# samuel-vitorino/sopro

Measured on AMD Instinct MI355X. Metric: audio_seconds_per_second, higher is better.
Workload: dtype f32; 1 GPU; Sopro-135M synthesize, 32 utterances x 200 frames per GPU (BASELINE configs[1]), S=64 text tokens, 32 distinct 150-frame reference voice(s) per batch prepared outside the timed region, top_p=0.9 T=1.05 anti_loop (reference defaults), synthetic weights with EOS suppressed; batch_per_gpu=32, frames=200, voices_per_batch=32, parallelism=replicas x1 (utterance sharding, no collective), lanes_per_gpu=4

## Files before the change

include/sopro_hip.h:

```cpp
#ifndef SOPRO_HIP_H
#define SOPRO_HIP_H

#include <stdint.h>

#ifdef __cplusplus
extern "C" {
#endif

#define SOPRO_ABI_VERSION 42

const char* sopro_last_error(void);
int sopro_abi_version(void);
int sopro_build_flags(void);
int sopro_set_lds_floor(int bytes);
int sopro_set_host_wait(int blocking);
int sopro_device_info(int device, int* out4);

int sopro_capture_begin(void* stream);
int sopro_capture_end(void* stream, void** graph_exec_out);
int sopro_graph_launch(void* graph_exec, void* stream);
int sopro_graph_launch_n(void* graph_exec, void* stream, int32_t n);
int sopro_graph_destroy(void* graph_exec);
int sopro_stream_create_cu_range(int first_cu, int n_cus, void** stream_out);
int sopro_stream_create_cu_mask(const uint32_t* mask, int32_t words, void** stream_out);
// ... 70 lines not shown
  long long* dbg;
  float eps;
  int32_t B, N, K, epilogue;
  int32_t ring_len, ring_bcap, dil, ksize;
  int32_t np, ksplit, rms_norm;
  int32_t w_layout;
  const float* aux_W; const float* aux_bias; const float* aux_R; float* aux_Y;
  int64_t aux_ldy, aux_ldr, aux_y_part_stride;
  int32_t aux_tiles, aux_flags;
  int32_t ring_format;
  int32_t mt, nt;
} sopro_skinny_args;
int sopro_skinny_f32(const sopro_skinny_args* args, void* stream);
int sopro_pack_skinny_w(const float* W, int64_t ldw, int32_t N, int32_t K, int32_t glu, float* out, void* stream);
int64_t sopro_skinny_packed_floats(int32_t N, int32_t K, int32_t glu);
int sopro_pack_skinny_w_bf16(const float* W, int64_t ldw, int32_t N, int32_t K, int32_t glu, void* out, void* stream);

int sopro_fill2d_u32(void* p, int64_t pitch, int32_t rows, int32_t width, uint32_t value, void* stream);
int sopro_copy2d_u32(void* dst, int64_t dpitch, const void* src, int64_t spitch, int32_t rows, int32_t width, void* stream);
int sopro_nar_seed_i32(int32_t* tokens, int32_t Q, const int32_t* cb0, int64_t cb0_bstride, int32_t B, int32_t T, int32_t vmax, void* stream);
int sopro_cvt_f32_bf16(const float* src, void* dst, int64_t n, void* stream);
int sopro_cvt_bf16_f32(const void* src, float* dst, int64_t n, void* stream);
enum { SOPRO_NORM_RMS = 0, SOPRO_NORM_LN = 1 };
int sopro_norm_f32(const float* x, int64_t ldx, int64_t x_seg_stride , float* out, int64_t ldo, const float* w, const float* b,
                   const float* mul, const float* add, int32_t rows, int32_t rows_per_seg, int32_t C,
                   float eps, int32_t kind, void* stream);
int sopro_row_stats_f32(const float* x, int64_t ldx, int64_t x_seg_stride , int32_t rows, int32_t rows_per_seg, int32_t C,
                        float* stats, void* stream);
int sopro_rms_match_f32(const float* a, const float* x, float* out, int32_t rows, int32_t C, void* stream);
int sopro_tanh_affine_f32(const float* in, float* out, float c0, float c1, int64_t n, void* stream);
int sopro_add_pos_f32(const float* rowvec, const float* table, float* out, int32_t B, int32_t T, int32_t C,
                      int32_t pos0, void* stream);
int sopro_masked_mean_f32(const float* x, const int32_t* lens, float* out, int32_t B, int32_t T, int32_t C,
                          void* stream);

int sopro_stats_pool_f32(const float* h, const float* logit, const int32_t* lens, float* out, int32_t B, int32_t T,
                         int32_t C, void* stream);
int sopro_l2norm_f32(const float* x, float* out, int32_t rows, int32_t C, float eps, void* stream);

int sopro_dwconv_f32(const float* x, const float* w, const float* bias, const float* res, float* out,
                     const int32_t* lens, int32_t B, int32_t T, int32_t C, int32_t ksize, int32_t dil,
                     int32_t left, int32_t mode, void* stream);

int sopro_codebook_sum_f32(const int32_t* tok, int32_t ldt, const int32_t* col, const int32_t* off, const float* wq,
                           int32_t nq, const float* table, int64_t table_rows, const float* base, float alpha,
                           float beta, float* out, int64_t ldo, int64_t o_seg_stride, int32_t rows,
                           int32_t rows_per_seg, int32_t D, void* stream);
int sopro_text_embed_f32(const int32_t* ids, const int32_t* lens, const float* table, int64_t table_rows,
                         const float* pe, float* out, int32_t B, int32_t T, int32_t C, void* stream);
int sopro_argmax_rows_f32(const float* x, int64_t ldx, int32_t* out, int64_t ldo, int32_t inner, int32_t rows, int32_t N,
                          void* stream);
int sopro_argmax_partials_i32(const float* partials, int64_t ldp, int32_t* out, int64_t ldo, int32_t heads, int32_t per_head, int32_t V,
                              int32_t rows, void* stream);

int sopro_fir1_f32(const float* x, int64_t x_seg_stride, int32_t n_in, const float* w, const float* bias, float* out,
                   int64_t ldo, int64_t o_seg_stride, int32_t B, int32_t n_out, int32_t C, int32_t K, int32_t stride,
                   int32_t left, void* stream);
int sopro_rvq_assign_f32(const float* scores, int64_t lds, int32_t V, const float* table, float* res, int64_t ldr,
                         int32_t D, int32_t* codes, int64_t ldc, int32_t rows, void* stream);

typedef struct sopro_attn_args {
  const float* Q; int64_t ldq; int64_t q_bstride;
  const float* K; int64_t ldk; int64_t k_bstride;
  const float* V; int64_t ldv; int64_t v_bstride;
  float* O; int64_t ldo; int64_t o_bstride;
  const int32_t* klens;
  int32_t B, H, dh, Tq, Tk;
  int32_t causal, q_pos0, k_pos0, window;
  float scale;
  const int32_t* kv_index;
} sopro_attn_args;
int sopro_attention_f32(const sopro_attn_args* args, void* stream);
int sopro_attention_split_bf16(const sopro_attn_args* args, int32_t passes, void* stream);
int sopro_attn_decode_f32(const sopro_attn_args* args, void* stream);
typedef struct sopro_xattn_args {
  const float* X; int64_t ldx;
  const float* Xp; int64_t xp_stride;
  const float* norm_w;
  const float* Kp; const float* Vp;
  const int32_t* klens;
  float* Y; int64_t y_part_stride;
  float eps, gate, scale;
  int32_t np, B, H, D, S_cap;
  const float* Qp; int64_t qp_stride;
  int32_t nqp, k_unfolded;
  int32_t kv_format;
} sopro_xattn_args;
int sopro_xattn_step_f32(const sopro_xattn_args* args, void* stream);

int sopro_rope_f32(float* x, int64_t ldx, const float* cos_t, const float* sin_t, int32_t rows,
                   int32_t rows_per_seg, int32_t pos0, int32_t H, int32_t dh, void* stream);

int sopro_upsample2_f32(const float* x, const float* w, float* y, int64_t y_seg_stride, int32_t B, int32_t T,
                        int32_t C, void* stream);
int sopro_final_conv_f32(const float* h, int64_t h_seg_stride, const float* w, float bias, float* wav,
                         int64_t wav_seg_stride, int32_t B, int32_t T, void* stream);

int sopro_seanet_tail_f32(const float* h, int64_t h_seg_stride, const float* w1, const float* b1, const float* w2,
                          const float* b2, const float* wf, float bf, float* wav, int64_t wav_seg_stride, int32_t B,
                          int32_t T, void* stream);
int sopro_seanet_tail_p_f32(const float* h, int64_t h_seg_stride, const float* w1, const float* b1, const float* w2,
                            const float* b2, const float* wf, float bf, float* wav, int64_t wav_seg_stride, int32_t B,
                            int32_t T, int32_t passes, void* stream);
int sopro_seanet_res128_f32(const float* h, int64_t h_seg_stride, const float* w1, const float* b1, const float* w2, const float* b2,
                            float* out, int64_t out_seg_stride, int32_t B, int32_t T, void* stream);
int sopro_seanet_res128_p_f32(const float* h, int64_t h_seg_stride, const float* w1, const float* b1, const float* w2, const float* b2,
// ... 214 lines not shown
```

sopro_amd/csrc/stages.hip:

```cpp
#include <stdlib.h>

#include <algorithm>
#include <map>
#include <string>
#include <vector>

#include "common.h"

int sopro_stream_batch_append(float* cur, float* other, const float* qkv, int32_t hs, int32_t rows, int64_t bstride, int32_t n, int32_t kv_len,
                              int32_t nkeep, hipStream_t s);
int sopro_stream_batch_gather(float* kv, const int32_t* keep, int32_t n_keep, int32_t layers, int32_t rows_cap, int64_t bstride, int32_t hs, int32_t half,
                              int32_t kv_len, hipStream_t s);

namespace {

struct Ten {
  const void* p = nullptr;
  int64_t shape[4] = {0, 0, 0, 0};
  int ndim = 0;
  const float* f() const { return reinterpret_cast<const float*>(p); }
};

struct Wt {
  const float* f32 = nullptr;
// ... 886 lines not shown
  for (int i = 0; i < c.n_layers_ar; ++i) {
    const int64_t n = (int64_t)((c.ar_kernel - 1) * c.ar_dilations[i] + 1) * B * D;
    STG(sopro_fill2d_u32(p.rings[i], n, 1, (int32_t)n, 0u, s));
  }
  STG(sopro_fill2d_u32(p.hist, (int64_t)B * Tar, 1, B * Tar, 0u, s));
  for (int k = 0; k < 8; ++k) {
    uint32_t u;
    memcpy(&u, &params[k], 4);
    STG(sopro_fill2d_u32(p.params + k, 1, 1, 1, u, s));
  }
  STG(sopro_fill2d_u32(p.nonce, B, 1, B, nonce, s));
  STG(sopro_fill2d_u32(p.key, 1, 1, 1, (uint32_t)seed, s));
  STG(sopro_fill2d_u32(p.key + 1, 1, 1, 1, (uint32_t)(seed >> 32), s));
  sopro_ar_state& st = p.st;
  memset(&st, 0, sizeof(st));
  st.x_cur = p.x[0]; st.cond = p.cond; st.emb = F(e, "cb_embed"); st.hist = p.hist;
  st.step = p.ctr; st.row_step = p.row_step; st.n_stopped = p.ctr + 2;
  st.first_eos = p.first_eos; st.stop_t = p.stop_t; st.recent = p.recent; st.params = p.params; st.nonce = p.nonce;
  st.key = p.key; st.seed = 0; st.B = B; st.D = D; st.Tar = Tar; st.max_steps = Tar; st.V = c.codebook_size; st.bos_row = c.bos_row;
  STG(sopro_ar_init(&st, s));
  if (p.graph && (p.graph_B != B || p.graph_S_cap != p.S_cap || p.graph_Tar != Tar || p.graph_ws != workspace)) {
    STG(sopro_graph_destroy(p.graph));
    p.graph = nullptr;
  }
  return 0;
}

int sopro_ar_run_graph(sopro_engine* e, int32_t n_steps, void* stream) {
  SOPRO_CHECK_ARG(e && e->ar.ws && n_steps >= 0 && stream, "sopro_ar_begin first; a non-default stream is needed for graph capture");
  ArPlan& p = e->ar;
  if (!p.graph) {
    STG(sopro_capture_begin(stream));
    const int rc = ar_issue_step(e, (hipStream_t)stream);
    void* g = nullptr;
    const int rc2 = sopro_capture_end(stream, &g);
    if (rc != 0) return rc;
    if (rc2 != 0) return rc2;
    p.graph = g; p.graph_B = p.B; p.graph_S_cap = p.S_cap; p.graph_Tar = p.Tar; p.graph_ws = p.ws;
  }
  for (int i = 0; i < n_steps; ++i) STG(sopro_graph_launch(p.graph, stream));
  return 0;
}

int sopro_ar_tokens(sopro_engine* e, int32_t* hist, int32_t* first_eos, int32_t* n_stopped, void* stream) {
  SOPRO_CHECK_ARG(e && e->ar.ws, "sopro_ar_begin first");
  hipStream_t s = (hipStream_t)stream;
  const ArPlan& p = e->ar;
  if (hist) STG(sopro_copy2d_u32(hist, (int64_t)p.B * p.Tar, p.hist, (int64_t)p.B * p.Tar, 1, p.B * p.Tar, s));
  if (first_eos) STG(sopro_copy2d_u32(first_eos, p.B, p.first_eos, p.B, 1, p.B, s));
  if (n_stopped) STG(sopro_copy2d_u32(n_stopped, 1, p.ctr + 2, 1, 1, 1, s));
  return 0;
}

struct NarWs { float *xa, *xb, *h, *x1, *u, *z, *part, *cond; int32_t *lens, *range; SplitK sk; };
static size_t nar_carve(const sopro_engine* e, NarWs& w, void* ws, int B, int T) {
  const sopro_engine_cfg& c = e->c;
  const size_t M = (size_t)B * T, D = c.d_model;
  int nh_max = 0;
  for (int i = 0; i < c.n_stages; ++i) nh_max = c.stage_n_cb[i] > nh_max ? c.stage_n_cb[i] : nh_max;
  Carver cv(ws);
  w.xa = cv.take<float>(M * D); w.xb = cv.take<float>(M * D); w.h = cv.take<float>(M * D); w.x1 = cv.take<float>(M * D);
  w.u = cv.take<float>(M * 4 * D); w.z = cv.take<float>(M * c.nar_head_dim);
  w.part = cv.take<float>(M * nh_max * (c.codebook_size / 64) * 2);
  w.cond = cv.take<float>(M * D);
  w.lens = cv.take<int32_t>(B);
  w.range = cv.take<int32_t>(4);
  w.sk.tickets = cv.take<int32_t>(SPLITK_TICKETS);
  w.sk.ws = M <= 1024 ? cv.take<float>(SPLITK_WS_BYTES / 4) : nullptr;
  return cv.off;
}

int64_t sopro_nar_workspace_bytes(const sopro_engine* e, int32_t B, int32_t T) {
  if (!e || B <= 0 || T <= 0) return 0;
  NarWs w;
  return (int64_t)nar_carve(e, w, nullptr, B, T);
}

static int ssm_block_bufs(sopro_engine* e, hipStream_t s, float* h, float* x1, float* u, const SplitK* sk, const float* x, float* out,
                          const std::string& p, int B, int T, int ksize, int dil, const int32_t* lens, const char* sfx, int32_t* range) {
  const int D = e->c.d_model, M = B * T;
  const int total = (ksize - 1) * dil, left = total / 2;
  G g; g.M = M; g.N = 2 * D; g.K = D; g.bias = F(e, p + ".glu.b"); g.epi = SOPRO_EPI_GLU; g.rms_eps = RMS_EPS; g.range_events = range;
  STG(gemm(s, x, WT(e, p + ".glu.wn" + sfx), nullptr, h, g));
  STG(sopro_dwconv_f32(h, F(e, p + ".dw.w"), F(e, p + ".dw.b"), x, x1, lens, B, T, D, ksize, dil, left, 1, s));
  G f1; f1.M = M; f1.N = 4 * D; f1.K = D; f1.bias = F(e, p + ".ff1.b"); f1.epi = SOPRO_EPI_GELU; f1.rms_eps = RMS_EPS; f1.range_events = range;
  STG(gemm(s, x1, WT(e, p + ".ff1.wn" + sfx), nullptr, u, f1));
  G f2; f2.M = M; f2.N = D; f2.K = 4 * D; f2.bias = F(e, p + ".ff2.b"); f2.epi = SOPRO_EPI_RES; f2.R = x1; f2.sk = sk; f2.range_events = range;
  return gemm(s, u, WT(e, p + ".ff2.w" + sfx), nullptr, out, f2);
}
static int ssm_block_seq(sopro_engine* e, hipStream_t s, const NarWs& w, const float* x, float* out, const std::string& p, int B, int T,
                         int ksize, int dil, const int32_t* lens, const char* sfx) {
  return ssm_block_bufs(e, s, w.h, w.x1, w.u, &w.sk, x, out, p, B, T, ksize, dil, lens, sfx, w.range);
}

int sopro_nar_refine_io(sopro_engine* e, void* workspace, const sopro_nar_io* io, int32_t B, int32_t T, void* stream) {
  SOPRO_CHECK_ARG(e && e->final && e->has_nar && workspace && io && io->cond && io->cb0 && io->tokens && B > 0 && T > 0,
                  "bad arguments (finalize the engine with the NAR tensors first)");
  hipStream_t s = (hipStream_t)stream;
  const sopro_engine_cfg& c = e->c;
  const int D = c.d_model, V = c.codebook_size, Q = c.num_codebooks, HD = c.nar_head_dim, M = B * T;
  SOPRO_CHECK_ARG(V % 64 == 0, "codebook_size must be a multiple of 64 (arg-max partials per 64 columns)");
  SOPRO_CHECK_ARG(io->cond_bstride >= (int64_t)T * D && io->cb0_bstride >= T, "cond / cb0 blocks shorter than T rows");
  const bool safe = io->safe != 0 && c.precision == 0;
  const char* sfx = safe ? NAR_SAFE : "";
  int32_t* tokens = io->tokens;
  NarWs w;
  nar_carve(e, w, workspace, B, T);
  if (w.sk.ws) STG(sopro_fill2d_u32(w.sk.tickets, SPLITK_TICKETS, 1, SPLITK_TICKETS, 0u, s));
  STG(sopro_fill2d_u32(w.range, 4, 1, 4, 0u, s));
  int nh_max = 0;
  for (int i = 0; i < c.n_stages; ++i) nh_max = c.stage_n_cb[i] > nh_max ? c.stage_n_cb[i] : nh_max;
  const float* cnd = io->cond;
  if (io->cond_bstride != (int64_t)T * D) {
    STG(sopro_copy2d_u32(w.cond, (int64_t)T * D, io->cond, io->cond_bstride, B, T * D, s));
    cnd = w.cond;
  }
  STG(sopro_nar_seed_i32(tokens, Q, io->cb0, io->cb0_bstride, B, T, V - 1, s));
  const int32_t* lens_d = nullptr;
  if (io->lens) {
    STG(sopro_copy2d_u32(w.lens, B, io->lens, B, 1, B, s));
    lens_d = w.lens;
  }
  const char* stage_names[8] = {"B", "C", "D", "E", "F", "G", "H", "I"};
  for (int sid = 0; sid < c.n_stages; ++sid) {
    float *xa = w.xa, *xb = w.xb;
    STG(sopro_codebook_sum_f32(tokens, Q, e->nar_cols[sid], e->nar_offs[sid], e->nar_cw[sid], e->nar_known[sid], F(e, "cb_embed"),
                               e->t["cb_embed"].shape[0], cnd, c.nar_mix[sid][0], c.nar_mix[sid][1], xa, D, 0, M, M, D, s));
    STG(norm(s, xa, xb, F(e, "nar.adapter.norm.weight"), M, D, RMS_EPS, SOPRO_NORM_RMS, nullptr, e->ad_mul[sid], e->ad_add[sid], M));
    std::swap(xa, xb);
    for (int i = 0; i < c.n_layers_nar; ++i) {
      STG(ssm_block_seq(e, s, w, xa, xb, "nar.blocks." + std::to_string(i), B, T, c.nar_kernel, c.nar_dilations[i], lens_d, sfx));
      std::swap(xa, xb);
    }
    STG(norm(s, xa, xb, F(e, "nar.norm.weight"), M, D, RMS_EPS));
    G pz; pz.M = M; pz.N = HD; pz.K = D; pz.bias = F(e, "nar.pre.b"); pz.range_events = w.range;
    STG(gemm(s, xb, WT(e, std::string("nar.pre.w") + sfx), nullptr, w.z, pz));
    const int nh = c.stage_n_cb[sid];
    const std::string hk = std::string("nar.heads.") + stage_names[sid];
    G hg; hg.M = M; hg.N = nh * V; hg.K = HD; hg.bias = F(e, hk + ".b"); hg.c_mode = 5; hg.C2 = w.part; hg.ldc2 = (int64_t)nh_max * (V / 64);
    hg.range_events = w.range;
    STG(gemm(s, w.z, WT(e, hk + ".w" + sfx), nullptr, nullptr, hg));
    STG(sopro_argmax_partials_i32(w.part, (int64_t)nh_max * (V / 64), tokens + c.stage_first_cb[sid], Q, nh, V / 64, V, M, s));
  }
  if (io->range_out) STG(sopro_copy2d_u32(io->range_out, 1, w.range, 1, 1, 1, s));
  return 0;
}

int sopro_nar_refine(sopro_engine* e, void* workspace, const float* cond, int64_t cond_bstride, const int32_t* rvq1, const int32_t* lens,
                     int32_t B, int32_t T, int32_t* tokens, void* stream) {
  sopro_nar_io io;
  memset(&io, 0, sizeof(io));
  io.cond = cond; io.cond_bstride = cond_bstride; io.cb0 = rvq1; io.cb0_bstride = T; io.lens = lens; io.tokens = tokens;
  return sopro_nar_refine_io(e, workspace, &io, B, T, stream);
}

struct MimiWs {
  int32_t* tok;
  float *emb, *q, *X, *y, *qkv, *ao, *hd, *e0, *hraw[8], *hact[8], *y1[8];
  float* lnst;
  SplitK sk;
};
static bool mimi_half(const sopro_engine* e) {
  static const bool off = getenv("SOPRO_MIMI_BF16") != nullptr && getenv("SOPRO_MIMI_BF16")[0] == '0';
  return e->c.precision == 1 && !off;
}

static bool seanet_fused(int B, int rows) {
  static const bool off = SOPRO_DEV_ENV("SOPRO_SEANET_FUSE") != nullptr && SOPRO_DEV_ENV("SOPRO_SEANET_FUSE")[0] == '0';
  return !off && (int64_t)B * rows >= 512 * 1024;
}

static size_t mimi_carve(const sopro_engine* e, MimiWs& w, void* ws, int B, int T) {
  const sopro_engine_cfg& c = e->c;
  const bool half = mimi_half(e);
  auto act = [&](Carver& cv_, size_t n) { return half ? reinterpret_cast<float*>(cv_.take<uint16_t>(n)) : cv_.take<float>(n); };
  const size_t HS = c.mimi_hidden, CD = c.mimi_codebook_dim, N2 = 2 * (size_t)T, PADX = c.mimi_kernel - 1;
  Carver cv(ws);
  w.tok = cv.take<int32_t>((size_t)B * T * c.num_codebooks);
  w.sk.tickets = cv.take<int32_t>(SPLITK_TICKETS);
  w.sk.ws = (size_t)B * N2 <= 512 ? cv.take<float>(SPLITK_WS_BYTES / 4) : nullptr;
  w.emb = cv.take<float>((size_t)B * T * 2 * CD);
  w.q = cv.take<float>((size_t)B * T * HS);
  w.X = cv.take<float>((size_t)B * (PADX + N2) * HS);
  w.y = cv.take<float>((size_t)B * N2 * HS);
  w.qkv = cv.take<float>((size_t)B * N2 * 3 * HS);
  w.ao = cv.take<float>((size_t)B * N2 * HS);
  w.hd = cv.take<float>((size_t)B * N2 * c.mimi_inter);
  w.lnst = cv.take<float>((size_t)B * N2 * ((HS + 63) / 64) * 2);
  size_t ch = (size_t)c.mimi_num_filters << c.mimi_n_ratios, rows = N2;
  w.e0 = act(cv, (size_t)B * (1 + rows) * ch);
  for (int si = 0; si < c.mimi_n_ratios; ++si) {
    const size_t co = ch / 2, orow = rows * c.mimi_ratios[si];
    const bool on_cu = si + 1 == c.mimi_n_ratios && ch == 128 && c.mimi_ratios[si] == 4 && seanet_fused(B, (int)rows);
    w.hraw[si] = on_cu ? nullptr : act(cv, (size_t)B * (2 + orow) * co);
// ... 495 lines not shown
```

sopro_amd/hip.py:

```python
from __future__ import annotations

import ctypes as C
import gc
import os
import threading
from typing import List, Optional

import torch

_HERE = os.path.dirname(os.path.abspath(__file__))
LIB_PATH = os.path.join(_HERE, "libsopro_hip.so")
ABI_VERSION = 42
DEV_MODE = os.environ.get("SOPRO_DEV", "0") == "1"


def dev_env(name: str, default: str) -> str:
    return os.environ.get(name, default) if DEV_MODE else default


DEFAULT_GROUP_M = 8
PRO_NONE, PRO_ELU, PRO_ADDVEC = 0, 1, 2
EPI_ROPE = 6
EPI_NONE, EPI_GELU, EPI_GLU, EPI_RES, EPI_TANH, EPI_GLU_DW = 0, 1, 2, 3, 4, 5
NORM_RMS, NORM_LN = 0, 1
# ... 107 lines not shown
    "sopro_capture_begin": (C.c_int, [_p]),
    "sopro_capture_end": (C.c_int, [_p, C.POINTER(_p)]),
    "sopro_graph_launch": (C.c_int, [_p, _p]),
    "sopro_graph_destroy": (C.c_int, [_p]),
    "sopro_stream_create_cu_range": (C.c_int, [C.c_int, C.c_int, C.POINTER(_p)]),
    "sopro_stream_create_cu_mask": (C.c_int, [_p, _i32, _p]),
    "sopro_stream_destroy": (C.c_int, [_p]),
    "sopro_gemm_f32": (C.c_int, [C.POINTER(GemmArgs), _p]),
    "sopro_gemm_bf16x3": (C.c_int, [_p, _p, _p, _p]),
    "sopro_gemm_bf16x6": (C.c_int, [_p, _p, _p, _p]),
    "sopro_gemm_bf16x1": (C.c_int, [_p, _p, _p, _p]),
    "sopro_pack_w_bf16": (C.c_int, [_p, _i64, _i32, _i32, _i32, _p, _p]),
    "sopro_fill2d_u32": (C.c_int, [_p, _i64, _i32, _i32, C.c_uint32, _p]),
    "sopro_copy2d_u32": (C.c_int, [_p, _i64, _p, _i64, _i32, _i32, _p]),
    "sopro_pack_w_f16x2": (C.c_int, [_p, _i64, _i32, _i32, _f32, _p, _p]),
    "sopro_f16x3_a_scale": (C.c_float, []),
    "sopro_gemm_f16x3": (C.c_int, [_p, _p, _p, _p]),
    "sopro_packed_w_bytes": (C.c_int64, [_i32, _i32, _i32]),
    "sopro_packed_w_rows_bytes": (C.c_int64, [_i32, _i32]),
    "sopro_pack_w_rows_bf16": (C.c_int, [_p, _i64, _i32, _i32, _p, _p]),
    "sopro_gemm_8p_takes": (C.c_int, [_p, _p]),
    "sopro_gemm_bf16x3_8p": (C.c_int, [_p, _p, _p, _p]),
    "sopro_gemm_bf16_set_tile_override": (C.c_int, [C.c_int]),
    "sopro_gemm_set_group_m": (C.c_int, [C.c_int]),
    "sopro_seanet_tail_set_tiles": (C.c_int, [C.c_int]),
    "sopro_seanet_res_set_tiles": (C.c_int, [C.c_int]),
    "sopro_seanet_res128_bf16": (C.c_int, [_p, _i64, _p, _p, _p, _p, _p, _i64, _i32, _i32, _p]),
    "sopro_seanet_up128_bf16": (C.c_int, [_p, _i64, _p, _p, _p, _i64, _i32, _i32, _p]),
    "sopro_seanet_tail_bf16": (C.c_int, [_p, _i64, _p, _p, _p, _p, _p, _f32, _p, _i64, _i32, _i32, _p]),
    "sopro_seanet_up_set_tiles": (C.c_int, [C.c_int]),
    "sopro_seanet_uptail_set_tiles": (C.c_int, [C.c_int]),
    "sopro_seanet_uptail_f32": (C.c_int, [_p, _i64, _p, _p, _p, _p, _p, _p, _p, _f32, _p, _i64, _i32, _i32, _i32, _p]),
    "sopro_seanet_uptail_bf16": (C.c_int, [_p, _i64, _p, _p, _p, _p, _p, _p, _p, _f32, _p, _i64, _i32, _i32, _p]),
    "sopro_seanet_up128_f32": (C.c_int, [_p, _i64, _p, _p, _p, _i64, _i32, _i32, _i32, _p]),
    "sopro_seanet_res128_f32": (C.c_int, [_p, _i64, _p, _p, _p, _p, _p, _i64, _i32, _i32, _p]),
    "sopro_gemm_set_tile_override": (C.c_int, [C.c_int]),
    "sopro_pack_skinny_w": (C.c_int, [_p, _i64, _i32, _i32, _i32, _p, _p]),
    "sopro_pack_skinny_w_bf16": (C.c_int, [_p, _i64, _i32, _i32, _i32, _p, _p]),
    "sopro_skinny_packed_floats": (_i64, [_i32, _i32, _i32]),
    "sopro_skinny_f32": (C.c_int, [C.POINTER(SkinnyArgs), _p]),
    "sopro_row_stats_f32": (C.c_int, [_p, _i64, _i64, _i32, _i32, _i32, _p, _p]),
    "sopro_norm_f32": (C.c_int, [_p, _i64, _i64, _p, _i64, _p, _p, _p, _p, _i32, _i32, _i32, _f32, _i32, _p]),
    "sopro_rms_match_f32": (C.c_int, [_p, _p, _p, _i32, _i32, _p]),
    "sopro_tanh_affine_f32": (C.c_int, [_p, _p, _f32, _f32, _i64, _p]),
    "sopro_add_pos_f32": (C.c_int, [_p, _p, _p, _i32, _i32, _i32, _i32, _p]),
    "sopro_masked_mean_f32": (C.c_int, [_p, _p, _p, _i32, _i32, _i32, _p]),
    "sopro_stats_pool_f32": (C.c_int, [_p, _p, _p, _p, _i32, _i32, _i32, _p]),
    "sopro_l2norm_f32": (C.c_int, [_p, _p, _i32, _i32, _f32, _p]),
    "sopro_dwconv_f32": (C.c_int, [_p, _p, _p, _p, _p, _p, _i32, _i32, _i32, _i32, _i32, _i32, _i32, _p]),
    "sopro_codebook_sum_f32": (C.c_int, [_p, _i32, _p, _p, _p, _i32, _p, _i64, _p, _f32, _f32, _p, _i64, _i64, _i32, _i32, _i32, _p]),
    "sopro_text_embed_f32": (C.c_int, [_p, _p, _p, _i64, _p, _p, _i32, _i32, _i32, _p]),
    "sopro_argmax_rows_f32": (C.c_int, [_p, _i64, _p, _i64, _i32, _i32, _i32, _p]),
    "sopro_argmax_partials_i32": (C.c_int, [_p, _i64, _p, _i64, _i32, _i32, _i32, _i32, _p]),
    "sopro_fir1_f32": (C.c_int, [_p, _i64, _i32, _p, _p, _p, _i64, _i64, _i32, _i32, _i32, _i32, _i32, _i32, _p]),
    "sopro_rvq_assign_f32": (C.c_int, [_p, _i64, _i32, _p, _p, _i64, _i32, _p, _i64, _i32, _p]),
    "sopro_attention_f32": (C.c_int, [C.POINTER(AttnArgs), _p]),
    "sopro_attention_split_bf16": (C.c_int, [C.POINTER(AttnArgs), C.c_int32, _p]),
    "sopro_attn_decode_f32": (C.c_int, [C.POINTER(AttnArgs), _p]),
    "sopro_xattn_step_f32": (C.c_int, [C.POINTER(XattnArgs), _p]),
    "sopro_rope_f32": (C.c_int, [_p, _i64, _p, _p, _i32, _i32, _i32, _i32, _i32, _p]),
    "sopro_upsample2_f32": (C.c_int, [_p, _p, _p, _i64, _i32, _i32, _i32, _p]),
    "sopro_final_conv_f32": (C.c_int, [_p, _i64, _p, _f32, _p, _i64, _i32, _i32, _p]),
    "sopro_seanet_tail_f32": (C.c_int, [_p, _i64, _p, _p, _p, _p, _p, _f32, _p, _i64, _i32, _i32, _p]),
    "sopro_seanet_res128_p_f32": (C.c_int, [_p, _i64, _p, _p, _p, _p, _p, _i64, _i32, _i32, _i32, _p]),
    "sopro_seanet_tail_p_f32": (C.c_int, [_p, _i64, _p, _p, _p, _p, _p, _f32, _p, _i64, _i32, _i32, _i32, _p]),
    "sopro_engine_create": (C.c_int, [C.POINTER(EngineCfg), C.POINTER(_p)]),
    "sopro_engine_set_tensor": (C.c_int, [_p, C.c_char_p, _p, C.POINTER(_i64), _i32]),
    "sopro_engine_finalize": (C.c_int, [_p, _p]),
    "sopro_engine_destroy": (C.c_int, [_p]),
    "sopro_ar_workspace_bytes": (_i64, [_p, _i32, _i32, _i32]),
    "sopro_ar_begin": (C.c_int, [_p, _p, _i32, _p, _p, _p, _i32, _i32, C.POINTER(_f32), C.c_uint64, C.c_uint32, _p]),
    "sopro_ar_run_graph": (C.c_int, [_p, _i32, _p]),
    "sopro_ar_tokens": (C.c_int, [_p, _p, _p, _p, _p]),
    "sopro_nar_workspace_bytes": (_i64, [_p, _i32, _i32]),
    "sopro_nar_refine": (C.c_int, [_p, _p, _p, _i64, _p, _p, _i32, _i32, _p, _p]),
    "sopro_nar_refine_io": (C.c_int, [_p, _p, C.POINTER(NarIO), _i32, _i32, _p]),
    "sopro_nar_seed_i32": (C.c_int, [_p, _i32, _p, _i64, _i32, _i32, _i32, _p]),
    "sopro_mimi_workspace_bytes": (_i64, [_p, _i32, _i32]),
    "sopro_mimi_decode": (C.c_int, [_p, _p, _p, _i32, _i32, _p, _p]),
    "sopro_mimi_chunk_rows": (_i32, [_i32, _i32]),
    "sopro_mimi_decode_parts": (C.c_int, [_p, _p, _p, _i32, _i32, _p, _i32, _p]),
    "sopro_mimi_stream_kv_bytes": (_i64, [_p, _i32]),
    "sopro_mimi_stream_init": (C.c_int, [_p, C.POINTER(MimiStreamState), _p, _i32]),
    "sopro_mimi_stream_trim": (C.c_int, [C.POINTER(MimiStreamState), _i32]),
    "sopro_mimi_decode_stream": (C.c_int, [_p, _p, C.POINTER(MimiStreamState), _p, _i32, _p, _p]),
    "sopro_mimi_stream_batch_kv_bytes": (_i64, [_p, _i32, _i32]),
    "sopro_mimi_stream_batch_init": (C.c_int, [_p, C.POINTER(MimiStreamBatch), _p, _i32, _i32]),
    "sopro_mimi_stream_batch_trim": (C.c_int, [C.POINTER(MimiStreamBatch), _i32]),
    "sopro_mimi_stream_batch_keep": (C.c_int, [_p, C.POINTER(MimiStreamBatch), C.POINTER(_i32), _i32, _p]),
    "sopro_mimi_decode_stream_batch": (C.c_int, [_p, _p, C.POINTER(MimiStreamBatch), _p, _i32, _p, _p]),
    "sopro_ar_init": (C.c_int, [C.POINTER(ArState), _p]),
    "sopro_ar_sample": (C.c_int, [C.POINTER(ArState), _p, _i64, _p]),
    "sopro_ar_admit": (C.c_int, [C.POINTER(ArState), _i32, _p]),
    "sopro_ar_issue_frame": (C.c_int, [C.POINTER(ArFrame), _p]),
    "sopro_ar_fold_text": (C.c_int, [_p, _p, _p, _p, _p, _p, _p, _p, _p, _i32, _i32, _i32, _i32, _i32, _f32, _p]),
    "sopro_ar_fold_text_uk": (C.c_int, [_p, _p, _p, _p, _p, _p, _p, _p, _i32, _i32, _i32, _i32, _i32, _f32, _p]),
    "sopro_engine_upload_tensor": (C.c_int, [_p, C.c_char_p, _p, C.POINTER(_i64), _i32, _p]),
    "sopro_checkpoint_open": (C.c_int, [C.c_char_p, C.c_char_p, C.POINTER(_p)]),
    "sopro_checkpoint_close": (C.c_int, [_p]),
    "sopro_checkpoint_count": (_i32, [_p]),
    "sopro_checkpoint_tensor": (C.c_int, [_p, _i32, C.POINTER(C.c_char_p), C.POINTER(_p), C.POINTER(_i64), C.POINTER(_i32)]),
    "sopro_checkpoint_engine_cfg": (C.c_int, [_p, _i32, C.POINTER(EngineCfg)]),
    "sopro_engine_from_checkpoint": (C.c_int, [_p, _i32, _p, C.POINTER(_p)]),
    "sopro_engine_set_ar_tiles": (C.c_int, [_p, _i32, _i32, _i32, _i32]),
    "sopro_cond_workspace_bytes": (_i64, [_p, _i32, _i32, _i32]),
    "sopro_cond_prepare": (C.c_int, [_p, _p, _p, _p, _i32, _p, _p, _p, _p, _i64, _p, _p, _i32, _i32, _i32, _i32, _p, _p, _p, _p]),
# ... 416 lines not shown


def add_pos(rowvec: torch.Tensor, table: torch.Tensor, out: torch.Tensor, B: int, T: int, C_: int, pos0: int = 0) -> None:
    _check(load().sopro_add_pos_f32(ptr(rowvec), ptr(table), ptr(out), B, T, C_, pos0, _stream()), "sopro_add_pos_f32")


def masked_mean(x: torch.Tensor, lens: Optional[torch.Tensor], out: torch.Tensor, B: int, T: int, C_: int) -> None:
    _check(load().sopro_masked_mean_f32(ptr(x), ptr(lens, torch.int32), ptr(out), B, T, C_, _stream()), "sopro_masked_mean_f32")


def stats_pool(h: torch.Tensor, logit: torch.Tensor, lens: Optional[torch.Tensor], out: torch.Tensor, B: int, T: int, C_: int) -> None:
    _check(load().sopro_stats_pool_f32(ptr(h), ptr(logit), ptr(lens, torch.int32), ptr(out), B, T, C_, _stream()), "sopro_stats_pool_f32")


def l2norm(x: torch.Tensor, out: torch.Tensor, rows: int, C_: int, eps: float = 1e-6) -> None:
    _check(load().sopro_l2norm_f32(ptr(x), ptr(out), rows, C_, eps, _stream()), "sopro_l2norm_f32")


def dwconv(x: torch.Tensor, w: torch.Tensor, bias: Optional[torch.Tensor], out: torch.Tensor, *, B: int, T: int, C_: int,
           ksize: int, dil: int, left: int, mode: int = 0, res: Optional[torch.Tensor] = None,
           lens: Optional[torch.Tensor] = None) -> None:
    _check(load().sopro_dwconv_f32(ptr(x), ptr(w), ptr(bias), ptr(res), ptr(out), ptr(lens, torch.int32), B, T, C_, ksize,
                                   dil, left, mode, _stream()), "sopro_dwconv_f32")


def codebook_sum(tok: torch.Tensor, ldt: int, col: torch.Tensor, off: torch.Tensor, wq: torch.Tensor, table: torch.Tensor,
                 out: torch.Tensor, *, rows: int, D: int, base: Optional[torch.Tensor] = None, alpha: float = 0.0,
                 beta: float = 1.0, ldo: Optional[int] = None, rows_per_seg: Optional[int] = None, o_seg_stride: int = 0,
                 o_off: int = 0, tok_off: int = 0) -> None:
    _check(load().sopro_codebook_sum_f32(ptr(tok, torch.int32) + 4 * tok_off, ldt, ptr(col, torch.int32), ptr(off, torch.int32),
                                         ptr(wq), int(col.numel()), ptr(table), int(table.shape[0]), ptr(base), alpha, beta,
                                         ptr(out) + 4 * o_off, D if ldo is None else ldo, o_seg_stride, rows,
                                         rows if rows_per_seg is None else rows_per_seg, D, _stream()), "sopro_codebook_sum_f32")


def text_embed(ids: torch.Tensor, lens: Optional[torch.Tensor], table: torch.Tensor, pe: torch.Tensor, out: torch.Tensor,
               B: int, T: int, C_: int) -> None:
    _check(load().sopro_text_embed_f32(ptr(ids, torch.int32), ptr(lens, torch.int32), ptr(table), int(table.shape[0]), ptr(pe),
                                       ptr(out), B, T, C_, _stream()), "sopro_text_embed_f32")


def argmax_rows(x: torch.Tensor, out: torch.Tensor, *, rows: int, N: int, ldx: Optional[int] = None, ldo: int = 1,
                o_off: int = 0, inner: int = 1) -> None:
    _check(load().sopro_argmax_rows_f32(ptr(x), N if ldx is None else ldx, ptr(out, torch.int32) + 4 * o_off, ldo, inner, rows, N,
                                        _stream()), "sopro_argmax_rows_f32")


def argmax_partials(part: torch.Tensor, out: torch.Tensor, *, rows: int, heads: int, per_head: int, V: int, ldp: int, ldo: int = 1,
                    o_off: int = 0) -> None:
    _check(load().sopro_argmax_partials_i32(ptr(part), ldp, ptr(out, torch.int32) + 4 * o_off, ldo, heads, per_head, V, rows, _stream()),
           "sopro_argmax_partials_i32")


def fir1(x: torch.Tensor, w: torch.Tensor, out: torch.Tensor, *, B: int, n_in: int, n_out: int, C_: int, K: int, stride: int,
         left: int, bias: Optional[torch.Tensor] = None, ldo: Optional[int] = None, x_seg_stride: Optional[int] = None,
         o_seg_stride: Optional[int] = None, o_off: int = 0) -> None:
    ldo = C_ if ldo is None else ldo
    _check(load().sopro_fir1_f32(ptr(x), n_in if x_seg_stride is None else x_seg_stride, n_in, ptr(w), ptr(bias) if bias is not None else None,
                                 ptr(out) + 4 * o_off, ldo, n_out * ldo if o_seg_stride is None else o_seg_stride, B, n_out, C_, K,
                                 stride, left, _stream()), "sopro_fir1_f32")


def rvq_assign(scores: torch.Tensor, table: torch.Tensor, res: torch.Tensor, codes: torch.Tensor, *, rows: int, V: int, D: int,
               ldc: int, t_off: int = 0, c_off: int = 0) -> None:
    _check(load().sopro_rvq_assign_f32(ptr(scores), V, V, ptr(table) + 4 * t_off, ptr(res), D, D, ptr(codes, torch.int32) + 4 * c_off,
                                       ldc, rows, _stream()), "sopro_rvq_assign_f32")


def attention(Q: torch.Tensor, K: torch.Tensor, V: torch.Tensor, O: torch.Tensor, *, B: int, H: int, dh: int, Tq: int,
              Tk: int, ldq: int, ldk: int, ldv: int, ldo: int, q_bstride: int, k_bstride: int, v_bstride: int,
              o_bstride: int, klens: Optional[torch.Tensor] = None, causal: bool = False, q_pos0: int = 0, k_pos0: int = 0,
              window: int = 0, scale: Optional[float] = None, q_off: int = 0, k_off: int = 0, v_off: int = 0,
              o_off: int = 0, decode: bool = False, kv_index: Optional[torch.Tensor] = None, split_passes: int = 0) -> None:
    a = AttnArgs()
    a.kv_index = ptr(kv_index, torch.int32)
    a.Q, a.ldq, a.q_bstride = ptr(Q) + 4 * q_off, ldq, q_bstride
    a.K, a.ldk, a.k_bstride = ptr(K) + 4 * k_off, ldk, k_bstride
    a.V, a.ldv, a.v_bstride = ptr(V) + 4 * v_off, ldv, v_bstride
    a.O, a.ldo, a.o_bstride = ptr(O) + 4 * o_off, ldo, o_bstride
    a.klens = ptr(klens, torch.int32)
    a.B, a.H, a.dh, a.Tq, a.Tk = B, H, dh, Tq, Tk
    a.causal, a.q_pos0, a.k_pos0, a.window = int(causal), q_pos0, k_pos0, window
    a.scale = float(scale if scale is not None else dh ** -0.5)
    if decode:
        _check(load().sopro_attn_decode_f32(C.byref(a), _stream()), "sopro_attn_decode_f32")
        return
    e0 = _prof.begin() if _prof is not None else None
    if split_passes:
        _check(load().sopro_attention_split_bf16(C.byref(a), int(split_passes), _stream()), "sopro_attention_split_bf16")
    else:
        _check(load().sopro_attention_f32(C.byref(a), _stream()), "sopro_attention_f32")
    if e0 is not None:
        pairs = float(Tq) * Tk if not causal else float(sum(max(0, min(Tk - 1, q_pos0 + q - k_pos0) - max(0, q_pos0 + q - window + 1 - k_pos0) + 1) for q in range(Tq)))
        _prof.end("attention_kernel", 4.0 * dh * pairs * B * H, e0)


def xattn_step(X: torch.Tensor, Y: torch.Tensor, norm_w: Optional[torch.Tensor], Kp: torch.Tensor, Vp: torch.Tensor, klens: Optional[torch.Tensor], *,
               B: int, H: int, D: int, S_cap: int, gate: float, scale: float, eps: float, Xp: Optional[torch.Tensor] = None, np_: int = 0,
               xp_stride: int = 0, y_part_stride: int = 0, Qp: Optional[torch.Tensor] = None, nqp: int = 0, qp_stride: int = 0) -> None:
    a = XattnArgs()
    if Qp is not None:
        a.Qp, a.nqp, a.qp_stride, a.k_unfolded = ptr(Qp), int(nqp), int(qp_stride), 1
    a.X, a.ldx, a.Xp, a.xp_stride, a.np = ptr(X), D, ptr(Xp), xp_stride, np_
    kv16 = Kp.dtype == torch.bfloat16
    a.norm_w, a.Kp, a.Vp, a.klens = ptr(norm_w), ptr(Kp, Kp.dtype), ptr(Vp, Kp.dtype), ptr(klens, torch.int32)
    a.kv_format = 1 if kv16 else 0
# ... 636 lines not shown
```

Measured before the change: 27680 audio-s/s.

## Fuse NAR head GEMM and argmax into one persistent f16x3 MFMA kernel

Adds a persistent kernel that computes the NAR codebook-head logits with split-f16 (three-pass) MFMA and reduces each row to an argmax in registers and LDS, writing tokens directly. This replaces the GEMM that wrote per-64-column partial maxima plus a separate argmax_partials launch. Work items (row block x head) are handed out through an atomic ticket counter, with the next activation block prefetched and staged into double-buffered LDS, and a weight-fragment queue. It is chosen only for f16-packed weights, default precision, K of 128 or 256, and enough items, and it adds a counter buffer and a custom tie-break path.

```diff
diff --git a/include/sopro_hip.h b/include/sopro_hip.h
--- a/include/sopro_hip.h
+++ b/include/sopro_hip.h
@@ -146,6 +146,10 @@
                           void* stream);
 int sopro_argmax_partials_i32(const float* partials, int64_t ldp, int32_t* out, int64_t ldo, int32_t heads, int32_t per_head, int32_t V,
                               int32_t rows, void* stream);
+int sopro_nar_heads_argmax_f16(const float* z, int64_t ldz, const void* packed_w, float acc_scale, const float* bias, int32_t* tokens,
+                               int64_t ldt, int32_t M, int32_t heads, int32_t V, int32_t K, int32_t* range_events, int32_t* work_ctr,
+                               void* stream);
+int sopro_nar_heads_set_form(int form);
 
 int sopro_fir1_f32(const float* x, int64_t x_seg_stride, int32_t n_in, const float* w, const float* bias, float* out,
                    int64_t ldo, int64_t o_seg_stride, int32_t B, int32_t n_out, int32_t C, int32_t K, int32_t stride,
diff --git a/sopro_amd/csrc/nar_heads.hip b/sopro_amd/csrc/nar_heads.hip
--- /dev/null
+++ b/sopro_amd/csrc/nar_heads.hip
@@ -0,0 +1,272 @@
+#include <math.h>
+
+#include "common.h"
+
+namespace {
+
+constexpr int NH_BM = 64, NH_BN = 256, NH_NT = 512, NH_D = 4;
+constexpr float NH_A16_SCALE = 8.0f;
+typedef _Float16 nh_f16x8 __attribute__((ext_vector_type(8)));
+typedef _Float16 nh_f16x2 __attribute__((ext_vector_type(2)));
+__device__ __forceinline__ nh_f16x8 nh_frag(const uint4& v) { return *reinterpret_cast<const nh_f16x8*>(&v); }
+__device__ __forceinline__ void nh_split_pair(float x, float y, unsigned& hi, unsigned& lo) {
+  const f32x2_t v = {x, y};
+  const nh_f16x2 h = __builtin_convertvector(v, nh_f16x2);
+  hi = *reinterpret_cast<const unsigned*>(&h);
+  const f32x2_t r = {x - (float)h[0], y - (float)h[1]};
+  const nh_f16x2 l = __builtin_convertvector(r, nh_f16x2);
+  lo = *reinterpret_cast<const unsigned*>(&l);
+}
+
+constexpr int NH_NONE_TILE = 0x7fffff;
+__device__ __forceinline__ void nh_take(float& bv, int& bc, float ov, int oc) {
+  const bool t = (ov > bv) | ((ov == bv) & (oc < bc));
+  bv = t ? ov : bv;
+  bc = t ? oc : bc;
+}
+
+template <int KS>
+__global__ __launch_bounds__(NH_NT, 1) void nar_heads_kernel(const float* __restrict__ z, int64_t ldz, const uint4* __restrict__ Wp, float cscale,
+                                                             const float* __restrict__ bias, int32_t* __restrict__ tokens, int64_t ldt, int M,
+                                                             int heads, int V, int32_t* __restrict__ range_events, int32_t* __restrict__ ctr,
+                                                             int order) {
+  constexpr int K = KS * 16;
+  constexpr int PITCH = K * 2 + 16;
+  constexpr int PLANE = NH_BM * PITCH;
+  constexpr int BUF = 2 * PLANE;
+  constexpr int F4ROW = K / 4;
+  constexpr int NLD = NH_BM * F4ROW / NH_NT;
+  static_assert((NH_BM * F4ROW) % NH_NT == 0 && KS % NH_D == 0, "staging / W queue");
+  extern __shared__ __attribute__((aligned(16))) unsigned char lds[];
+  float2* red = reinterpret_cast<float2*>(lds + 2 * BUF);
+  int* tk = reinterpret_cast<int*>(lds + 2 * BUF + 2 * 8 * NH_BM * (int)sizeof(float2));
+  const int tid = threadIdx.x, lane = tid & 63, wave = tid >> 6;
+  const int nmb = (M + NH_BM - 1) / NH_BM, nitems = nmb * heads, ntile = V / NH_BN;
+
+  if (tid == 0) {
+    const int t0 = atomicAdd(ctr, 1);
+    tk[2] = t0;
+    tk[0] = t0 < nitems ? atomicAdd(ctr, 1) : nitems;
+  }
+  __syncthreads();
+  int cur = tk[2];
+
+  float a16max = 0.f;
+  float4 v[NLD];
+  auto item_of = [&](int it, int& head, int& m0) {
+    if (order == 0) { head = it / nmb; m0 = (it - head * nmb) * NH_BM; }
+    else { const int mb = it / heads; head = it - mb * heads; m0 = mb * NH_BM; }
+  };
+  auto request = [&](int it) {
+    int head, m0;
+    item_of(it, head, m0);
+#pragma unroll
+    for (int i = 0; i < NLD; ++i) {
+      const int f = tid + i * NH_NT;
+      const int row = f / F4ROW, c4 = f - row * F4ROW;
+      v[i] = *reinterpret_cast<const float4*>(z + (int64_t)min(m0 + row, M - 1) * ldz + c4 * 4);
+    }
+  };
+  auto stage = [&](int buf) {
+    const float F16MAX = 65504.0f;
+#pragma unroll
+    for (int i = 0; i < NLD; ++i) {
+      const int f = tid + i * NH_NT;
+      const int row = f / F4ROW, c4 = f - row * F4ROW;
+      const float vx = v[i].x * NH_A16_SCALE, vy = v[i].y * NH_A16_SCALE, vz = v[i].z * NH_A16_SCALE, vw = v[i].w * NH_A16_SCALE;
+      a16max = fmaxf(a16max, fmaxf(fmaxf(fabsf(vx), fabsf(vy)), fmaxf(fabsf(vz), fabsf(vw))));
+      uint2 hi, lo;
+      nh_split_pair(__builtin_amdgcn_fmed3f(vx, -F16MAX, F16MAX), __builtin_amdgcn_fmed3f(vy, -F16MAX, F16MAX), hi.x, lo.x);
+      nh_split_pair(__builtin_amdgcn_fmed3f(vz, -F16MAX, F16MAX), __builtin_amdgcn_fmed3f(vw, -F16MAX, F16MAX), hi.y, lo.y);
+      unsigned char* p = lds + buf * BUF + row * PITCH + c4 * 8;
+      *reinterpret_cast<uint2*>(p) = hi;
+      *reinterpret_cast<uint2*>(p + PLANE) = lo;
+    }
+  };
+
+  if (cur < nitems) {
+    request(cur);
+    stage(0);
+  }
+  __syncthreads();
+
+  const int frow = lane & 31, fg = lane >> 5;
+  for (int n = 0; cur < nitems; ++n) {
+    const int buf = n & 1;
+    const int nxt = tk[n & 1];
+    const bool has_next = nxt < nitems;
+    int tk_next = nitems;
+    if (tid == 0 && has_next) tk_next = atomicAdd(ctr, 1);
+    int head, m0;
+    item_of(cur, head, m0);
+    head = __builtin_amdgcn_readfirstlane(head);
+    if (has_next) request(nxt);
+
+    const int wv = __builtin_amdgcn_readfirstlane(wave);
+    auto wtile = [&](int ct) -> const uint4* { return Wp + ((int64_t)(head * (V >> 5) + ct * (NH_BN / 32) + wv) * KS * 2) * 64; };
+    uint4 wq[NH_D][2];
+    {
+      const uint4* w0 = wtile(0);
+#pragma unroll
+      for (int d = 0; d < NH_D; ++d) {
+        wq[d][0] = w0[lane + (d * 2 + 0) * 64];
+        wq[d][1] = w0[lane + (d * 2 + 1) * 64];
+      }
+    }
+    const float* bhead = bias + (int64_t)head * V + wave * 32 + frow;
+    const unsigned char* abase = lds + buf * BUF + frow * PITCH + fg * 16;
+    float bv[32];
+    int bt[32];
+#pragma unroll
+    for (int r = 0; r < 32; ++r) { bv[r] = -INFINITY; bt[r] = NH_NONE_TILE; }
+
+    for (int ct = 0; ct < ntile; ++ct) {
+      f32x16 acc[2];
+#pragma unroll
+      for (int i = 0; i < 2; ++i)
+#pragma unroll
+        for (int r = 0; r < 16; ++r) acc[i][r] = 0.f;
+      const uint4* wcur = wtile(ct);
+      const uint4* wnxt = wtile(min(ct + 1, ntile - 1));
+      const float bcol = bhead[ct * NH_BN];
+      uint4 ah[2], al[2];
+#pragma unroll
+      for (int i = 0; i < 2; ++i) {
+        ah[i] = *reinterpret_cast<const uint4*>(abase + i * 32 * PITCH);
+        al[i] = *reinterpret_cast<const uint4*>(abase + i * 32 * PITCH + PLANE);
+      }
+#pragma unroll
+      for (int s = 0; s < KS; ++s) {
+        const uint4 wh = wq[s % NH_D][0], wl = wq[s % NH_D][1];
+        {
+          const int sn = s + NH_D;
+          const uint4* src = sn < KS ? wcur : wnxt;
+          const int so = (sn < KS ? sn : sn - KS) * 2 * 64;
+          wq[s % NH_D][0] = src[lane + so];
+          wq[s % NH_D][1] = src[lane + so + 64];
+        }
+        __builtin_amdgcn_sched_barrier(0);
+        const uint4 ch0 = ah[0], ch1 = ah[1], cl0 = al[0], cl1 = al[1];
+        if (s + 1 < KS) {
+#pragma unroll
+          for (int i = 0; i < 2; ++i) {
+            ah[i] = *reinterpret_cast<const uint4*>(abase + i * 32 * PITCH + (s + 1) * 32);
+            al[i] = *reinterpret_cast<const uint4*>(abase + i * 32 * PITCH + (s + 1) * 32 + PLANE);
+          }
+        }
+        acc[0] = __builtin_amdgcn_mfma_f32_32x32x16_f16(nh_frag(cl0), nh_frag(wh), acc[0], 0, 0, 0);
+        acc[1] = __builtin_amdgcn_mfma_f32_32x32x16_f16(nh_frag(cl1), nh_frag(wh), acc[1], 0, 0, 0);
+        acc[0] = __builtin_amdgcn_mfma_f32_32x32x16_f16(nh_frag(ch0), nh_frag(wl), acc[0], 0, 0, 0);
+        acc[1] = __builtin_amdgcn_mfma_f32_32x32x16_f16(nh_frag(ch1), nh_frag(wl), acc[1], 0, 0, 0);
+        acc[0] = __builtin_amdgcn_mfma_f32_32x32x16_f16(nh_frag(ch0), nh_frag(wh), acc[0], 0, 0, 0);
+        acc[1] = __builtin_amdgcn_mfma_f32_32x32x16_f16(nh_frag(ch1), nh_frag(wh), acc[1], 0, 0, 0);
+        __builtin_amdgcn_sched_barrier(0);
+      }
+#pragma unroll
+      for (int i = 0; i < 2; ++i)
+#pragma unroll
+        for (int q = 0; q < 16; ++q) {
+          const float lg = acc[i][q] * cscale + bcol;
+          const bool t = lg > bv[i * 16 + q];
+          bv[i * 16 + q] = t ? lg : bv[i * 16 + q];
+          bt[i * 16 + q] = t ? ct : bt[i * 16 + q];
+        }
+      if (ct == 0 && has_next) stage(buf ^ 1);
+    }
+
+    const int cbase = wave * 32 + frow;
+#pragma unroll
+    for (int r = 0; r < 32; ++r) bt[r] = bt[r] * NH_BN + cbase;
+#pragma unroll
+    for (int h = 16; h >= 1; h >>= 1) {
+      const bool up = (frow & h) != 0;
+#pragma unroll
+      for (int j = 0; j < h; ++j) {
+        float v0 = bv[j], v1 = bv[j + h];
+        int c0 = bt[j], c1 = bt[j + h];
+        asm volatile("" : "+v"(v0), "+v"(v1), "+v"(c0), "+v"(c1));
+        const float sv = up ? v0 : v1;
+        const int sc = up ? c0 : c1;
+        float kv = up ? v1 : v0;
+        int kc = up ? c1 : c0;
+        nh_take(kv, kc, __shfl_xor(sv, h, 64), __shfl_xor(sc, h, 64));
+        bv[j] = kv;
+        bt[j] = kc;
+      }
+    }
+    const int rrow = 32 * (frow >> 4) + 8 * ((frow & 15) >> 2) + 4 * fg + (frow & 3);
+    float2* rd = red + (n & 1) * 8 * NH_BM;
+    rd[wave * NH_BM + rrow] = make_float2(bv[0], __int_as_float(bt[0]));
+    if (tid == 0) tk[(n + 1) & 1] = tk_next;
+    __syncthreads();
+    if (tid < NH_BM) {
+      float best = -INFINITY;
+      int bc = NH_NONE_TILE * NH_BN;
+#pragma unroll
+      for (int w8 = 0; w8 < 8; ++w8) {
+        const float2 p = rd[w8 * NH_BM + tid];
+        nh_take(best, bc, p.x, __float_as_int(p.y));
+      }
+      if (m0 + tid < M) tokens[(int64_t)(m0 + tid) * ldt + head] = bc < V ? bc : 0;
+    }
+    cur = nxt;
+  }
+  if (range_events && !(a16max <= 65504.0f)) atomicAdd(range_events, 1);
+  if (tid == 0) {
+    const int old = __hip_atomic_fetch_add(ctr + 1, 1, __ATOMIC_ACQ_REL, __HIP_MEMORY_SCOPE_AGENT);
+    if (old == (int)gridDim.x - 1) {
+      __hip_atomic_store(ctr, 0, __ATOMIC_RELAXED, __HIP_MEMORY_SCOPE_AGENT);
+      __hip_atomic_store(ctr + 1, 0, __ATOMIC_RELAXED, __HIP_MEMORY_SCOPE_AGENT);
+    }
+  }
+}
+
+template <int KS>
+int nh_launch(const float* z, int64_t ldz, const uint4* wp, float cscale, const float* bias, int32_t* tokens, int64_t ldt, int M, int heads,
+              int V, int32_t* range_events, int32_t* ctr, int order, hipStream_t s) {
+  constexpr size_t lds = (size_t)2 * 2 * NH_BM * (KS * 32 + 16) + (size_t)2 * 8 * NH_BM * sizeof(float2) + 16;
+  auto kern = nar_heads_kernel<KS>;
+  SOPRO_SET_MAX_LDS_ONCE(kern, lds);
+  static int n_cu[64] = {};
+  int dev = 0;
+  SOPRO_HIP(hipGetDevice(&dev));
+  if (!n_cu[dev & 63]) {
+    hipDeviceProp_t p;
+    SOPRO_HIP(hipGetDeviceProperties(&p, dev));
+    n_cu[dev & 63] = p.multiProcessorCount > 0 ? p.multiProcessorCount : 1;
+  }
+  const int64_t nitems = (int64_t)((M + NH_BM - 1) / NH_BM) * heads;
+  const unsigned grid = (unsigned)(nitems < n_cu[dev & 63] ? nitems : n_cu[dev & 63]);
+  hipLaunchKernelGGL(kern, dim3(grid), dim3(NH_NT), lds, s, z, ldz, wp, cscale, bias, tokens, ldt, M, heads, V, range_events, ctr, order);
+  SOPRO_LAUNCH_CHECK();
+}
+
+int g_nar_heads_form = 0;
+
+}
+
+extern "C" int sopro_nar_heads_set_form(int form) {
+  g_nar_heads_form = form >= 0 && form <= 3 ? form : 0;
+  return 0;
+}
+
+int sopro_nar_heads_form(void) { return g_nar_heads_form; }
+
+extern "C" int sopro_nar_heads_argmax_f16(const float* z, int64_t ldz, const void* packed_w, float acc_scale, const float* bias, int32_t* tokens,
+                                          int64_t ldt, int32_t M, int32_t heads, int32_t V, int32_t K, int32_t* range_events, int32_t* work_ctr,
+                                          void* stream) {
+  SOPRO_CHECK_ARG(z && packed_w && bias && tokens && work_ctr, "z, packed_w, bias, tokens, work_ctr must be non-NULL");
+  SOPRO_CHECK_ARG(M > 0 && heads > 0 && V > 0 && (int64_t)heads * V < ((int64_t)1 << 30), "M, heads, V must be positive (heads x V < 2^30)");
+  SOPRO_CHECK_ARG(K == 128 || K == 256, "K must be 128 or 256 (the rows of a block stay in LDS)");
+  SOPRO_CHECK_ARG(V % NH_BN == 0, "V must be a multiple of 256 (column tiles)");
+  SOPRO_CHECK_ARG(ldz >= K && (ldz & 3) == 0 && aligned16(z) && aligned16(packed_w), "z rows and packed_w must be 16-byte aligned, ldz >= K");
+  SOPRO_CHECK_ARG(ldt >= heads, "ldt must hold the heads");
+  int ex = 0;
+  SOPRO_CHECK_ARG(acc_scale > 0.f && frexpf(acc_scale, &ex) == 0.5f, "acc_scale must be a power of two (1 / (activation scale x pack scale))");
+  SOPRO_CHECK_ARG(sopro_f16x3_a_scale() == NH_A16_SCALE, "the activation scale of this kernel differs from sopro_f16x3_a_scale()");
+  const uint4* wp = reinterpret_cast<const uint4*>(packed_w);
+  const int order = g_nar_heads_form == 3 ? 1 : 0;
+  hipStream_t s = reinterpret_cast<hipStream_t>(stream);
+  if (K == 256) return nh_launch<16>(z, ldz, wp, acc_scale, bias, tokens, ldt, M, heads, V, range_events, work_ctr, order, s);
+  return nh_launch<8>(z, ldz, wp, acc_scale, bias, tokens, ldt, M, heads, V, range_events, work_ctr, order, s);
+}
diff --git a/sopro_amd/csrc/stages.hip b/sopro_amd/csrc/stages.hip
--- a/sopro_amd/csrc/stages.hip
+++ b/sopro_amd/csrc/stages.hip
@@ -962,7 +962,7 @@
   return 0;
 }
 
-struct NarWs { float *xa, *xb, *h, *x1, *u, *z, *part, *cond; int32_t *lens, *range; SplitK sk; };
+struct NarWs { float *xa, *xb, *h, *x1, *u, *z, *part, *cond; int32_t *lens, *range, *hctr; SplitK sk; };
 static size_t nar_carve(const sopro_engine* e, NarWs& w, void* ws, int B, int T) {
   const sopro_engine_cfg& c = e->c;
   const size_t M = (size_t)B * T, D = c.d_model;
@@ -975,6 +975,7 @@
   w.cond = cv.take<float>(M * D);
   w.lens = cv.take<int32_t>(B);
   w.range = cv.take<int32_t>(4);
+  w.hctr = cv.take<int32_t>(4);
   w.sk.tickets = cv.take<int32_t>(SPLITK_TICKETS);
   w.sk.ws = M <= 1024 ? cv.take<float>(SPLITK_WS_BYTES / 4) : nullptr;
   return cv.off;
@@ -1001,6 +1002,14 @@
 static int ssm_block_seq(sopro_engine* e, hipStream_t s, const NarWs& w, const float* x, float* out, const std::string& p, int B, int T,
                          int ksize, int dil, const int32_t* lens, const char* sfx) {
   return ssm_block_bufs(e, s, w.h, w.x1, w.u, &w.sk, x, out, p, B, T, ksize, dil, lens, sfx, w.range);
+}
+
+extern "C++" int sopro_nar_heads_form(void);
+constexpr int NAR_HEADS_MIN_ITEMS = 256;
+static bool nar_heads_one_launch(const Wt& hw, bool safe, int precision, int HD, int V, int M, int nh) {
+  const int form = sopro_nar_heads_form();
+  if (form == 1 || precision != 0 || safe || !hw.packed || !hw.f16 || !(HD == 128 || HD == 256) || V % 256 != 0) return false;
+  return form >= 2 || (int64_t)((M + 63) / 64) * nh >= NAR_HEADS_MIN_ITEMS;
 }
 
 int sopro_nar_refine_io(sopro_engine* e, void* workspace, const sopro_nar_io* io, int32_t B, int32_t T, void* stream) {
@@ -1018,6 +1027,7 @@
   nar_carve(e, w, workspace, B, T);
   if (w.sk.ws) STG(sopro_fill2d_u32(w.sk.tickets, SPLITK_TICKETS, 1, SPLITK_TICKETS, 0u, s));
   STG(sopro_fill2d_u32(w.range, 4, 1, 4, 0u, s));
+  STG(sopro_fill2d_u32(w.hctr, 4, 1, 4, 0u, s));
   int nh_max = 0;
   for (int i = 0; i < c.n_stages; ++i) nh_max = c.stage_n_cb[i] > nh_max ? c.stage_n_cb[i] : nh_max;
   const float* cnd = io->cond;
@@ -1047,9 +1057,16 @@
     STG(gemm(s, xb, WT(e, std::string("nar.pre.w") + sfx), nullptr, w.z, pz));
     const int nh = c.stage_n_cb[sid];
     const std::string hk = std::string("nar.heads.") + stage_names[sid];
+    const Wt& hw = WT(e, hk + ".w" + sfx);
+    if (nar_heads_one_launch(hw, safe, c.precision, HD, V, M, nh)) {
+      sopro_prof_scope prof("gemm_f16x3_kernel", 2.0 * M * nh * V * HD, s);
+      STG(sopro_nar_heads_argmax_f16(w.z, HD, hw.packed, hw.acc_scale, F(e, hk + ".b"), tokens + c.stage_first_cb[sid], Q, M, nh, V, HD, w.range,
+                                     w.hctr, s));
+      continue;
+    }
     G hg; hg.M = M; hg.N = nh * V; hg.K = HD; hg.bias = F(e, hk + ".b"); hg.c_mode = 5; hg.C2 = w.part; hg.ldc2 = (int64_t)nh_max * (V / 64);
     hg.range_events = w.range;
-    STG(gemm(s, w.z, WT(e, hk + ".w" + sfx), nullptr, nullptr, hg));
+    STG(gemm(s, w.z, hw, nullptr, nullptr, hg));
     STG(sopro_argmax_partials_i32(w.part, (int64_t)nh_max * (V / 64), tokens + c.stage_first_cb[sid], Q, nh, V / 64, V, M, s));
   }
   if (io->range_out) STG(sopro_copy2d_u32(io->range_out, 1, w.range, 1, 1, 1, s));
diff --git a/sopro_amd/hip.py b/sopro_amd/hip.py
--- a/sopro_amd/hip.py
+++ b/sopro_amd/hip.py
@@ -183,6 +183,8 @@
     "sopro_text_embed_f32": (C.c_int, [_p, _p, _p, _i64, _p, _p, _i32, _i32, _i32, _p]),
     "sopro_argmax_rows_f32": (C.c_int, [_p, _i64, _p, _i64, _i32, _i32, _i32, _p]),
     "sopro_argmax_partials_i32": (C.c_int, [_p, _i64, _p, _i64, _i32, _i32, _i32, _i32, _p]),
+    "sopro_nar_heads_argmax_f16": (C.c_int, [_p, _i64, _p, _f32, _p, _p, _i64, _i32, _i32, _i32, _i32, _p, _p, _p]),
+    "sopro_nar_heads_set_form": (C.c_int, [C.c_int]),
     "sopro_fir1_f32": (C.c_int, [_p, _i64, _i32, _p, _p, _p, _i64, _i64, _i32, _i32, _i32, _i32, _i32, _i32, _p]),
     "sopro_rvq_assign_f32": (C.c_int, [_p, _i64, _i32, _p, _p, _i64, _i32, _p, _i64, _i32, _p]),
     "sopro_attention_f32": (C.c_int, [C.POINTER(AttnArgs), _p]),
@@ -705,6 +707,21 @@
            "sopro_argmax_partials_i32")
 
 
+def nar_heads_argmax(z: torch.Tensor, W: "PackedW", bias: torch.Tensor, tokens: torch.Tensor, work_ctr: torch.Tensor, *, M: int, heads: int,
+                     V: int, ldz: Optional[int] = None, ldt: Optional[int] = None, t_off: int = 0,
+                     range_events: Optional[torch.Tensor] = None) -> None:
+    if not (isinstance(W, PackedW) and W.f16) or W.N != heads * V:
+        raise SoproHipError("nar_heads_argmax wants the f16 three-pass packing (pack_w_f16x3) of the [heads * V, K] matrix")
+    _check(load().sopro_nar_heads_argmax_f16(ptr(z), W.K if ldz is None else ldz, ptr(W.data, torch.int32), W.acc_scale, ptr(bias),
+                                             ptr(tokens, torch.int32) + 4 * t_off, heads if ldt is None else ldt, M, heads, V, W.K,
+                                             ptr(range_events, torch.int32), ptr(work_ctr, torch.int32), _stream()),
+           "sopro_nar_heads_argmax_f16")
+
+
+def nar_heads_set_form(form: int) -> None:
+    _check(load().sopro_nar_heads_set_form(int(form)), "sopro_nar_heads_set_form")
+
+
 def fir1(x: torch.Tensor, w: torch.Tensor, out: torch.Tensor, *, B: int, n_in: int, n_out: int, C_: int, K: int, stride: int,
          left: int, bias: Optional[torch.Tensor] = None, ldo: Optional[int] = None, x_seg_stride: Optional[int] = None,
          o_seg_stride: Optional[int] = None, o_off: int = 0) -> None:
```

Measured after the change: 27570 audio-s/s. No clear change (-0.4%).
